# DiamondLightSource/volume-segmantics

Hardware: AMD Instinct MI355X
Metric: slices/sec fwd+bwd U-Net/ResNet-34 256x256 bf16 batch 32 (training step incl. loss, AdamW) (higher is better)
Workload: dtype bf16; 1 GPU; configs[1]: synthetic 256^3-style 1-ch slices, 2-class, U-Net/ResNet-34, batch 32 per GPU, train step (fwd + DiceLoss + bwd + AdamW + OneCycleLR); global_batch=32, slice=256x256, parallelism=dp1, master_weights=fp32

## Files before the change

### volume-segmantics_amd/csrc/conv_igemm.hip

```cpp
#include <hip/hip_fp16.h>

#include <algorithm>
#include <cstdlib>

#include "conv_common.h"
#include "conv_stream.h"
#include "prof.h"

namespace {

constexpr int kPS = 64;
__device__ __forceinline__ int swz(int row, int key, int seg) { return row * kPS + ((seg ^ ((key >> 1) & 3)) << 4); }


struct TileGeom {
    int tw_shift;
    int TH;
    int tiles_h, tiles_w;
    int PH, PW;
    int out_nchw;
    unsigned pw_magic, tw_magic;
    int groups, ctiles;
    unsigned ct_magic, ti_magic;
    unsigned long long* probe;
};

constexpr int patch_items(int pt, int stride, int nw = 4) {
    return nw == 8 ? 3 : (stride == 2 ? (pt == 2 ? 9 : 5) : (pt == 4 ? 6 : (pt == 2 ? 3 : 2)));
}

template <typename T, int BN, int PT, int NTAPS, int STRIDE, int NW = 4, int DIL = 1, bool NLOAD = false>
__global__ __launch_bounds__(NW * 64, NW == 8 ? 4 : 1) void conv_igemm_kernel(ConvParams p, TileGeom g) {
    constexpr int NT = NW * 64;
    constexpr int CK = CT<T>::CK, EPS = CT<T>::EPS;
    constexpr int NJ = BN / 16, KW = NTAPS == 9 ? 3 : 1;
    constexpr int PITEMS = patch_items(PT, DIL > 1 ? 2 : STRIDE, NW);
    constexpr int WROWS = NT / 4;
    constexpr int TS = WROWS / BN;
    static_assert(WROWS % BN == 0, "cout tile must divide the rows of a staging pass");
    constexpr int WITEMS = (NTAPS + TS - 1) / TS;
    extern __shared__ __attribute__((aligned(16))) char smem[];
    const int tid = threadIdx.x, lane = tid & 63, wave = tid >> 6;
    const int lq = lane >> 4, lr = lane & 15;
    constexpr bool kStatic = STRIDE == 1 && DIL == 1;
    constexpr int kTWS = PT == 1 ? 3 : 4, kTW = 1 << kTWS, kTH = NW * 16 * PT / kTW, kKH = NTAPS == 9 ? 3 : 1;
    const int tw_shift = kStatic ? kTWS : g.tw_shift;
    const int TW = 1 << tw_shift;
    const int PW = kStatic ? kTW - 1 + KW : g.PW;
    const int PH = kStatic ? kTH - 1 + kKH : g.PH;
    const int TH = kStatic ? kTH : g.TH;
    const int Cin = p.C0 + p.C1;
    const int P = PH * PW;
    char* patch = smem;
    char* wl = smem + P * kPS;
    asm volatile("" ::"s"(p.src0), "s"(p.src1), "s"(p.w), "s"(p.out), "s"(p.C0), "s"(p.C1), "s"(p.up0), "s"(p.Hin), "s"(p.Win),
                 "s"(p.Hout), "s"(p.Wout), "s"(p.pad), "s"(p.Cout), "s"(g.tiles_w), "s"(g.tw_magic), "s"(g.pw_magic), "s"(g.PW),
                 "s"(g.PH), "s"(g.tw_shift), "s"(g.probe), "s"(p.gc));
    unsigned long long tprobe[5];
    if (g.probe) tprobe[0] = wall_clock64();

    const int xcd = blockIdx.x & 7, slot = blockIdx.x >> 3;
    const int gl = g.ctiles == 1 ? slot : (int)__umulhi((unsigned)slot, g.ct_magic);
    const int ytile = slot - gl * g.ctiles;
    const int grp = gl * 8 + xcd;
    if (grp >= g.groups) return;
    const int tiles_img = g.tiles_h * g.tiles_w;
    const int n = tiles_img == 1 ? grp : (int)__umulhi((unsigned)grp, g.ti_magic);
    const int timg = grp - n * tiles_img;
    const int ty = g.tiles_w == 1 ? timg : (int)__umulhi((unsigned)timg, g.tw_magic);
    const int tx = timg - ty * g.tiles_w;
    const int h0 = ty * TH, w0 = tx * TW;
    const int n0 = ytile * BN;
    const int hbase = h0 * STRIDE - p.pad, wbase = w0 * STRIDE - p.pad;
    const int ush = p.up0 ? 1 : 0;
    const bool stuffed = p.up0 == 2;
    const int H0 = p.Hin >> ush, W0 = p.Win >> ush;
    const __amdgpu_buffer_rsrc_t r0 = __builtin_amdgcn_make_buffer_rsrc(
        (void*)((const T*)p.src0 + (size_t)n * H0 * W0 * p.C0), 0, H0 * W0 * p.C0 * (int)sizeof(T), 0x00020000);
    const __amdgpu_buffer_rsrc_t r1 = __builtin_amdgcn_make_buffer_rsrc(
        (void*)((const T*)p.src1 + (size_t)n * p.Hin * p.Win * p.C1), 0, p.src1 ? p.Hin * p.Win * p.C1 * (int)sizeof(T) : 0, 0x00020000);
    const int kbeg = p.gc ? n0 : 0, kend = p.gc ? n0 + p.gc : Cin;
    const int CinW = p.gc ? p.gc : Cin;
    const __amdgpu_buffer_rsrc_t rw = __builtin_amdgcn_make_buffer_rsrc((void*)p.w, 0, p.Cout * NTAPS * CinW * (int)sizeof(T), 0x00020000);
    const int dummy = (P + NTAPS * BN) * kPS;
    float* cst = reinterpret_cast<float*>(smem + dummy + 64);
    const int C0r = (p.C0 + 31) & ~31;
    if constexpr (NLOAD) {
        const long long* bins = reinterpret_cast<const long long*>(p.nl_bins);
        const double rows = (double)p.nl_rows;
        for (int ch = tid; ch < p.C0; ch += NT) {
            long long sv = 0, qv = 0;
#pragma unroll 8
// ... 94 lines not shown
                    float nm[8], na[8], nb[8];
#pragma unroll
                    for (int h = 0; h < 2; ++h) {
                        const float4 m4 = *reinterpret_cast<const float4*>(q + 4 * h), a4 = *reinterpret_cast<const float4*>(q + C0r + 4 * h),
                                     b4 = *reinterpret_cast<const float4*>(q + 2 * C0r + 4 * h);
                        nm[4 * h] = m4.x; nm[4 * h + 1] = m4.y; nm[4 * h + 2] = m4.z; nm[4 * h + 3] = m4.w;
                        na[4 * h] = a4.x; na[4 * h + 1] = a4.y; na[4 * h + 2] = a4.z; na[4 * h + 3] = a4.w;
                        nb[4 * h] = b4.x; nb[4 * h + 1] = b4.y; nb[4 * h + 2] = b4.z; nb[4 * h + 3] = b4.w;
                    }
                    const bool segok = (tid & 3) * EPS < p.C0 - c0;
#pragma unroll
                    for (int i = 0; i < PITEMS; ++i) pregs[s][i] = nl_apply8(pregs[s][i], segok && poff0[i] >= 0, nm, na, nb);
                    if (p.nl_y && ytile == (c0 / CK) % g.ctiles) {
                        const __amdgpu_buffer_rsrc_t ry = __builtin_amdgcn_make_buffer_rsrc(
                            (void*)((T*)p.nl_y + (size_t)n * H0 * W0 * p.C0), 0, H0 * W0 * p.C0 * (int)sizeof(T), 0x00020000);
#pragma unroll
                        for (int i = 0; i < PITEMS; ++i) {
                            const uint4 v = pregs[s][i];
                            __builtin_amdgcn_raw_buffer_store_b128(u32x4{v.x, v.y, v.z, v.w}, ry, (segok && ((ystore >> i) & 1u)) ? poff0[i] : (int)0x80000000,
                                                                   c0 * (int)sizeof(T), 0);
                        }
                    }
                }
            }
#pragma unroll
            for (int i = 0; i < PITEMS; ++i) *reinterpret_cast<uint4*>(patch + pdst[i]) = pregs[s][i];
#pragma unroll
            for (int i = 0; i < WITEMS; ++i) {
                const bool full = (i + 1) * TS <= NTAPS;
                const int dst = (full || wtap0 + i * TS < NTAPS) ? P * kPS + wdst0 + i * WROWS * kPS : dummy;
                *reinterpret_cast<uint4*>(smem + dst) = wregs[s][i];
            }
            __syncthreads();
            if (g.probe && c0 == kbeg) tprobe[2] = wall_clock64();
            if (c0 + PF * CK < kend) load_chunk(c0 + PF * CK, pregs[s], wregs[s]);
            uint4 wf[2][NJ], xf[2][PT];
            auto read_frags = [&](int tap, uint4 (&w)[NJ], uint4 (&x)[PT]) {
                const int kh = tap / KW, kw = tap % KW;
#pragma unroll
                for (int j = 0; j < NJ; ++j) w[j] = *reinterpret_cast<const uint4*>(wl + (tap * BN + j * 16) * kPS + wbase_l);
#pragma unroll
                for (int i = 0; i < PT; ++i) x[i] = *reinterpret_cast<const uint4*>(patch + xb[i][kw] + kh * khs);
            };
            constexpr int kMfmaPerTap = NJ * PT * (sizeof(T) == 2 ? 1 : 4);
            read_frags(0, wf[0], xf[0]);
            constexpr bool kPin = BN <= 32;
            if (kPin) __builtin_amdgcn_sched_group_barrier(0x100, NJ + PT, 0);
#pragma unroll
            for (int tap = 0; tap < NTAPS; ++tap) {
                if (tap + 1 < NTAPS) read_frags(tap + 1, wf[(tap + 1) & 1], xf[(tap + 1) & 1]);
#pragma unroll
                for (int i = 0; i < PT; ++i)
#pragma unroll
                    for (int j = 0; j < NJ; ++j) mma16<T>(acc[i][j], wf[tap & 1][j], xf[tap & 1][i]);
                if (kPin && tap + 1 < NTAPS) __builtin_amdgcn_sched_group_barrier(0x100, NJ + PT, 0);
                if (kPin) __builtin_amdgcn_sched_group_barrier(0x008, kMfmaPerTap, 0);
            }
        }
    }

    if (g.probe) tprobe[3] = wall_clock64();
    conv_epilogue<T, BN, PT, NW>(p, tw_shift, g.out_nchw, n, h0, w0, n0, grp, acc, smem);
    if (g.probe) {
        __builtin_amdgcn_s_waitcnt(0);
        tprobe[4] = wall_clock64();
        if (tid == 0) {
            unsigned long long* o = g.probe + (size_t)blockIdx.x * 8;
            for (int i = 0; i < 5; ++i) o[i] = tprobe[i];
            unsigned hw, xcc;
            asm volatile("s_getreg_b32 %0, hwreg(HW_REG_HW_ID)" : "=s"(hw));
            asm volatile("s_getreg_b32 %0, hwreg(HW_REG_XCC_ID)" : "=s"(xcc));
            o[5] = hw; o[6] = xcc; o[7] = 0;
        }
    }
}

struct DirectGeom {
    int strips_w, chunks_h, RH;
    unsigned sw_magic, ch_magic;
    int nwaves, out_nchw;
    int xcd;
};

template <typename T, int BN, int MODE>
__global__ __launch_bounds__(256, 4) void conv_direct_kernel(ConvParams p, DirectGeom g) {
    constexpr int EPS = CT<T>::EPS, NJ = BN / 16, NTAPS = 9, kD = (BN == 32 && MODE == 1) ? 2 : ((BN == 16 && MODE == 0) ? 2 : 4);
    constexpr int WTOTAL = NTAPS * BN * 4, WITEMS = (WTOTAL + 255) / 256;
    constexpr int kOob = (int)0x80000000;
    __shared__ __attribute__((aligned(16))) char wl[NTAPS * BN * kPS + 64];
    asm volatile("" ::"s"(p.src0), "s"(p.w), "s"(p.out), "s"(p.C0), "s"(p.up0), "s"(p.Hin), "s"(p.Win), "s"(p.Hout), "s"(p.Wout),
                 "s"(p.Cout), "s"(p.scale), "s"(p.shift), "s"(p.relu), "s"(p.stats_partial), "s"(g.strips_w), "s"(g.chunks_h),
                 "s"(g.RH), "s"(g.sw_magic), "s"(g.ch_magic), "s"(g.nwaves));
    const int tid = threadIdx.x, lane = tid & 63, wave = tid >> 6;
    const int lq = lane >> 4, lr = lane & 15;
    const int Cin = p.C0;
    {
        const __amdgpu_buffer_rsrc_t rw = make_rsrc(p.w, p.Cout * NTAPS * Cin * (int)sizeof(T));
#pragma unroll
        for (int i = 0; i < WITEMS; ++i) {
            const int item = tid + i * 256;
            const int row = item >> 2, seg = item & 3;
            const int tap = row / BN, nr = row % BN;
            const bool ok = item < WTOTAL && nr < p.Cout && seg * EPS < Cin;
            const uint4 v = bload(rw, ok ? ((nr * NTAPS + tap) * Cin + seg * EPS) * (int)sizeof(T) : -1, 0);
            *reinterpret_cast<uint4*>(wl + (item < WTOTAL ? swz(row, row, seg) : NTAPS * BN * kPS)) = v;
        }
    }
    __syncthreads();
    const int gw = xcd_block(g.xcd) * 4 + wave;
    if (gw >= g.nwaves) return;
    const int q = g.strips_w == 1 ? gw : (int)__umulhi((unsigned)gw, g.sw_magic);
    const int ws = gw - q * g.strips_w;
    const int n = g.chunks_h == 1 ? q : (int)__umulhi((unsigned)q, g.ch_magic);
    const int hc = q - n * g.chunks_h;
    const int w0 = ws * 16, h0 = hc * g.RH, h1 = min(p.Hout, h0 + g.RH);
    const int H0 = p.Hin >> p.up0, W0 = p.Win >> p.up0;
    const int rowbytes = W0 * p.C0 * (int)sizeof(T);
    const __amdgpu_buffer_rsrc_t rx = make_rsrc((const T*)p.src0 + (size_t)n * H0 * W0 * p.C0, H0 * rowbytes);
    int coff[3];
#pragma unroll
    for (int kw = 0; kw < 3; ++kw) {
        const int col = w0 + lr + kw - 1;
        coff[kw] = (col >= 0 && col < p.Win && lq * EPS < Cin) ? ((col >> p.up0) * p.C0 + lq * EPS) * (int)sizeof(T) : -1;
    }
    const int wbase_l = swz(lr, lr, lq);
    auto load_row = [&](int hi, uint4 (&x)[3]) {
        const bool ok = hi >= 0 && hi < p.Hin;
        const int soff = ok ? (hi >> p.up0) * rowbytes : 0;
#pragma unroll
        for (int kw = 0; kw < 3; ++kw) x[kw] = bload(rx, ok ? coff[kw] : -1, soff);
    };

    const int wo = w0 + lr;
    const bool inw = wo < p.Wout;
    __amdgpu_buffer_rsrc_t ro;
    int ooff[NJ], orow;
    if constexpr (MODE == 0) {
        ro = make_rsrc((T*)p.out + (size_t)n * p.Hout * p.Wout * p.Cout, p.Hout * p.Wout * p.Cout * (int)sizeof(T));
        orow = p.Wout * p.Cout * (int)sizeof(T);
#pragma unroll
        for (int j = 0; j < NJ; ++j) ooff[j] = (inw && j * 16 + lq * 4 < p.Cout) ? (wo * p.Cout + j * 16 + lq * 4) * (int)sizeof(T) : kOob;
    } else {
        const int Ho = p.Hout >> 1, Wo = p.Wout >> 1;
        ro = make_rsrc((T*)p.out + (size_t)n * Ho * Wo * p.Cout, Ho * Wo * p.Cout * (int)sizeof(T));
        orow = Wo * p.Cout * (int)sizeof(T);
#pragma unroll
        for (int j = 0; j < NJ; ++j)
            ooff[j] = (inw && !(lr & 1) && j * 16 + lq * 4 < p.Cout) ? ((wo >> 1) * p.Cout + j * 16 + lq * 4) * (int)sizeof(T) : kOob;
    }
    float4 sc[NJ], sh[NJ];
#pragma unroll
    for (int j = 0; j < NJ; ++j) {
        const int c = j * 16 + lq * 4;
        sc[j] = make_float4(1.f, 1.f, 1.f, 1.f); sh[j] = make_float4(0.f, 0.f, 0.f, 0.f);
        if (MODE != 1) {
            float a[4] = {1.f, 1.f, 1.f, 1.f}, b[4] = {0.f, 0.f, 0.f, 0.f};
#pragma unroll
            for (int r = 0; r < 4; ++r)
                if (c + r < p.Cout) { if (p.scale) a[r] = p.scale[c + r]; if (p.shift) b[r] = p.shift[c + r]; }
            sc[j] = make_float4(a[0], a[1], a[2], a[3]); sh[j] = make_float4(b[0], b[1], b[2], b[3]);
        }
    }
    const bool affine = MODE != 1 && (p.scale || p.shift);
    float s1[NJ][4], s2[NJ][4];
    f32x4 prev[NJ];
#pragma unroll
    for (int j = 0; j < NJ; ++j) {
        prev[j] = f32x4{0.f, 0.f, 0.f, 0.f};
#pragma unroll
        for (int r = 0; r < 4; ++r) s1[j][r] = s2[j][r] = 0.f;
    }

    f32x4 a0[NJ], a1[NJ], a2[NJ];
#pragma unroll
    for (int j = 0; j < NJ; ++j) a0[j] = a1[j] = a2[j] = f32x4{0.f, 0.f, 0.f, 0.f};
    uint4 ring[kD][3];
#pragma unroll
    for (int u = 0; u < kD; ++u) load_row(h0 - 1 + u, ring[u]);
    for (int base = h0 - 1; base <= h1; base += kD) {
#pragma unroll
        for (int u = 0; u < kD; ++u) {
            const int hi = base + u;
            if (hi > h1) break;
            int wb = wbase_l;
            if (NJ > 1 || MODE != 0) asm volatile("" : "+v"(wb));
#pragma unroll
            for (int kw = 0; kw < 3; ++kw)
#pragma unroll
                for (int j = 0; j < NJ; ++j) {
                    const uint4 w0f = *reinterpret_cast<const uint4*>(wl + ((0 * 3 + kw) * BN + j * 16) * kPS + wb);
                    const uint4 w1f = *reinterpret_cast<const uint4*>(wl + ((1 * 3 + kw) * BN + j * 16) * kPS + wb);
                    const uint4 w2f = *reinterpret_cast<const uint4*>(wl + ((2 * 3 + kw) * BN + j * 16) * kPS + wb);
                    mma16<T>(a2[j], w0f, ring[u][kw]);
                    mma16<T>(a1[j], w1f, ring[u][kw]);
                    mma16<T>(a0[j], w2f, ring[u][kw]);
                }
            load_row(hi + kD, ring[u]);
            const int h = hi - 1;
            const bool live = h >= h0;
#pragma unroll
            for (int j = 0; j < NJ; ++j) {
                if (MODE == 0 && (p.stats_partial || p.stats_bins) && live && inw) {
#pragma unroll
                    for (int r = 0; r < 4; ++r) { s1[j][r] += a0[j][r]; s2[j][r] += a0[j][r] * a0[j][r]; }
                }
                float v[4] = {a0[j][0], a0[j][1], a0[j][2], a0[j][3]};
                if constexpr (MODE == 1) {
#pragma unroll
                    for (int r = 0; r < 4; ++r) { v[r] += prev[j][r]; v[r] += __shfl_xor(v[r], 1, 64); }
                    prev[j] = a0[j];
                    const int off = (live && (h & 1)) ? ooff[j] : kOob;
                    uint2 pk;
                    if constexpr (sizeof(T) == 2) {
                        pk.x = pack2<T>(v[0], v[1]);
                        pk.y = pack2<T>(v[2], v[3]);
                        __builtin_amdgcn_raw_buffer_store_b64(__builtin_bit_cast(__attribute__((ext_vector_type(2))) unsigned int, pk), ro, off, (h >> 1) * orow, 0);
                    } else {
                        __builtin_amdgcn_raw_buffer_store_b128(u32x4{__float_as_uint(v[0]), __float_as_uint(v[1]), __float_as_uint(v[2]), __float_as_uint(v[3])}, ro, off, (h >> 1) * orow, 0);
                    }
                } else {
                    if (affine) {
                        v[0] = v[0] * sc[j].x + sh[j].x; v[1] = v[1] * sc[j].y + sh[j].y;
                        v[2] = v[2] * sc[j].z + sh[j].z; v[3] = v[3] * sc[j].w + sh[j].w;
                    }
                    if (p.relu == 1) { v[0] = fmaxf(v[0], 0.f); v[1] = fmaxf(v[1], 0.f); v[2] = fmaxf(v[2], 0.f); v[3] = fmaxf(v[3], 0.f); }
                    else if (p.relu == 2) {
#pragma unroll
                        for (int r = 0; r < 4; ++r) v[r] = v[r] / (1.f + __expf(-v[r]));
                    }
                    if constexpr (MODE == 0) {
                        const int off = live ? ooff[j] : kOob;
                        if constexpr (sizeof(T) == 2) {
                            uint2 pk;
                            pk.x = pack2<T>(v[0], v[1]);
                            pk.y = pack2<T>(v[2], v[3]);
                            __builtin_amdgcn_raw_buffer_store_b64(__builtin_bit_cast(__attribute__((ext_vector_type(2))) unsigned int, pk), ro, off, h * orow, 0);
                        } else {
                            __builtin_amdgcn_raw_buffer_store_b128(u32x4{__float_as_uint(v[0]), __float_as_uint(v[1]), __float_as_uint(v[2]), __float_as_uint(v[3])}, ro, off, h * orow, 0);
                        }
                    }
                }
            }
#pragma unroll
            for (int j = 0; j < NJ; ++j) { a0[j] = a1[j]; a1[j] = a2[j]; a2[j] = f32x4{0.f, 0.f, 0.f, 0.f}; }
        }
    }
    if (MODE == 0 && (p.stats_partial || p.stats_bins)) {
#pragma unroll
        for (int j = 0; j < NJ; ++j)
#pragma unroll
            for (int r = 0; r < 4; ++r) {
#pragma unroll
                for (int o = 1; o < 16; o <<= 1) { s1[j][r] += __shfl_xor(s1[j][r], o, 64); s2[j][r] += __shfl_xor(s2[j][r], o, 64); }
                const int c = j * 16 + lq * 4 + r;
                if (lr == 0 && c < p.Cout) {
                    if (p.stats_bins) {
                        unsigned long long* b = p.stats_bins + (size_t)(gw & (p.stats_nb - 1)) * 2 * p.Cout + c;
                        atomicAdd(b, (unsigned long long)__double2ll_rn((double)s1[j][r] * kStatScale1));
                        atomicAdd(b + p.Cout, (unsigned long long)__double2ll_rn((double)s2[j][r] * kStatScale2));
                    } else {
                        p.stats_partial[((size_t)gw * 2 + 0) * p.Cout + c] = s1[j][r];
                        p.stats_partial[((size_t)gw * 2 + 1) * p.Cout + c] = s2[j][r];
                    }
                }
            }
    }
}

template <typename T, int NK>
__global__ __launch_bounds__(256, 4) void head_dgrad_planes_kernel(const float* __restrict__ dl, const T* __restrict__ w, T* __restrict__ out, int N, int classes,
                                                                  int H, int W, int C, DirectGeom g) {
    constexpr int kOob = (int)0x80000000;
    const int tid = threadIdx.x, lane = tid & 63, wave = tid >> 6;
    const int lq = lane >> 4, lr = lane & 15;
    const int gw = blockIdx.x * 4 + wave;
    if (gw >= g.nwaves) return;
    const int q = g.strips_w == 1 ? gw : (int)__umulhi((unsigned)gw, g.sw_magic);
    const int ws = gw - q * g.strips_w;
    const int n = g.chunks_h == 1 ? q : (int)__umulhi((unsigned)q, g.ch_magic);
    const int hc = q - n * g.chunks_h;
    const int x = ws * 16 + lr, h0 = hc * g.RH, h1 = min(H, h0 + g.RH);
    const int KK = 9 * classes;
    uint4 af[NK];
    int poff[NK][8];
    int prow[NK][8];
#pragma unroll
    for (int qq = 0; qq < NK; ++qq) {
        unsigned short a8[8];
#pragma unroll
        for (int j = 0; j < 8; ++j) {
            const int kk = 32 * qq + 8 * lq + j;
            const bool live = kk < KK;
            const int t = live ? kk / classes : 0, k = live ? kk - t * classes : 0;
            const int r = t / 3, sft = t - 3 * r;
            a8[j] = (live && lr < C) ? __builtin_bit_cast(unsigned short, w[((size_t)k * 9 + t) * C + lr]) : (unsigned short)0;
            const int xx = x + 1 - sft;
            poff[qq][j] = (live && xx >= 0 && xx < W) ? k * H * W + (1 - r) * W + xx : kOob;
            prow[qq][j] = r;
        }
        af[qq] = make_uint4((unsigned)a8[0] | ((unsigned)a8[1] << 16), (unsigned)a8[2] | ((unsigned)a8[3] << 16),
                            (unsigned)a8[4] | ((unsigned)a8[5] << 16), (unsigned)a8[6] | ((unsigned)a8[7] << 16));
    }
    const float* dn = dl + (size_t)n * classes * H * W;
    const __amdgpu_buffer_rsrc_t ro = make_rsrc(out + (size_t)n * H * W * C, H * W * C * (int)sizeof(T));
    const int ooff = (x < W && lq * 4 < C) ? (x * C + lq * 4) * (int)sizeof(T) : kOob;
    auto gather = [&](int y, float (&v)[NK][8]) {
        bool rok[3];
#pragma unroll
        for (int r = 0; r < 3; ++r) { const int yy = y + 1 - r; rok[r] = yy >= 0 && yy < H && y < h1; }
#pragma unroll
        for (int qq = 0; qq < NK; ++qq)
#pragma unroll
            for (int j = 0; j < 8; ++j) {
                const bool ok = poff[qq][j] != kOob && rok[prow[qq][j]];
                v[qq][j] = ok ? dn[(size_t)y * W + poff[qq][j]] : 0.f;
            }
    };
    float cur[NK][8], nxt[NK][8];
    gather(h0, cur);
    for (int y = h0; y < h1; ++y) {
        gather(y + 1, nxt);
        f32x4 acc = f32x4{0.f, 0.f, 0.f, 0.f};
#pragma unroll
        for (int qq = 0; qq < NK; ++qq) {
            uint4 b;
            b.x = pack2<T>(cur[qq][0], cur[qq][1]); b.y = pack2<T>(cur[qq][2], cur[qq][3]);
            b.z = pack2<T>(cur[qq][4], cur[qq][5]); b.w = pack2<T>(cur[qq][6], cur[qq][7]);
            mma16<T>(acc, af[qq], b);
        }
        uint2 pk;
        pk.x = pack2<T>(acc[0], acc[1]);
        pk.y = pack2<T>(acc[2], acc[3]);
        __builtin_amdgcn_raw_buffer_store_b64(__builtin_bit_cast(__attribute__((ext_vector_type(2))) unsigned int, pk), ro, ooff, y * W * C * (int)sizeof(T), 0);
#pragma unroll
        for (int qq = 0; qq < NK; ++qq)
#pragma unroll
            for (int j = 0; j < 8; ++j) cur[qq][j] = nxt[qq][j];
    }
}
// ... 190 lines not shown
        coff[kw] = (col >= 0 && col < p.Win && lq * EPS < Cin) ? (col * p.C0 + lq * EPS) * (int)sizeof(T) : -1;
    }
    auto load_row = [&](int hi, uint4 (&x)[3]) {
        const bool ok = hi >= 0 && hi < p.Hin;
        const int soff = ok ? hi * rowbytes : 0;
#pragma unroll
        for (int kw = 0; kw < 3; ++kw) x[kw] = bload(rx, ok ? coff[kw] : -1, soff);
    };
    const int wbase_l = swz(lr, lr, lq);
    const int wo = w0 + lr;
    const bool inw = wo < p.Wout;
    float bias[4];
#pragma unroll
    for (int r = 0; r < 4; ++r) bias[r] = (p.shift && r < K) ? p.shift[r] : 0.f;
    const int plane = p.Hout * p.Wout * 4;
    const __amdgpu_buffer_rsrc_t ro = MODE == 2 ? make_rsrc((float*)p.out + (size_t)n * K * p.Hout * p.Wout, K * plane) : make_rsrc(nullptr, 0);

    f32x4 acc = f32x4{0.f, 0.f, 0.f, 0.f}, done = f32x4{0.f, 0.f, 0.f, 0.f};
    uint4 ring[kD][3];
#pragma unroll
    for (int u = 0; u < kD; ++u) load_row(h0 - 1 + u, ring[u]);
    for (int base = h0 - 1; base <= h1r; base += kD) {
#pragma unroll
        for (int u = 0; u < kD; ++u) {
            const int hi = base + u;
            if (hi > h1r) break;
            const int m = (u + 3) & 3;
            int wb = wbase_l;
            asm volatile("" : "+v"(wb));
#pragma unroll
            for (int kw = 0; kw < 3; ++kw)
                mma16<T>(acc, *reinterpret_cast<const uint4*>(wl + (m * 3 + kw) * 16 * kPS + wb), ring[u][kw]);
            load_row(hi + kD, ring[u]);
            const int qd = (u + 2) & 3;
            if (lq == qd) { done = acc; acc = f32x4{0.f, 0.f, 0.f, 0.f}; }
            if (qd == 3) {
                const int h = hi - 4 + lq;
                const bool live = h >= h0 && h < h1 && inw;
                float v[4];
#pragma unroll
                for (int r = 0; r < 4; ++r) v[r] = done[r] + bias[r];
                if constexpr (MODE == 2) {
#pragma unroll
                    for (int r = 0; r < 4; ++r)
                        __builtin_amdgcn_raw_buffer_store_b32(__float_as_uint(v[r]), ro, (live && r < K) ? (h * p.Wout + wo) * 4 : kOob, r * plane, 0);
                } else {
                    float mx = v[0];
#pragma unroll
                    for (int r = 1; r < 4; ++r) if (r < K) mx = fmaxf(mx, v[r]);
                    float sum = 0.f;
#pragma unroll
                    for (int r = 0; r < 4; ++r) if (r < K) sum += expf(v[r] - mx);
                    float best = -1.f;
                    int lab = 0;
#pragma unroll
                    for (int r = 0; r < 4; ++r)
                        if (r < K) { const float pk = __fdiv_rn(expf(v[r] - mx), sum); if (pk > best) { best = pk; lab = r; } }
                    const int rr = h - vsc.m.crop_top, jj = wo - vsc.m.crop_left;
                    if (live && rr >= 0 && rr < vsc.m.h && jj >= 0 && jj < vsc.m.w) {
                        const int64_t addr = vsc.m.base + (int64_t)(vsc.s0 + n) * vsc.m.ss + (int64_t)rr * vsc.m.sh + (int64_t)jj * vsc.m.sw;
                        const __half hv = __float2half_rn(best);
                        const uint32_t hb = __builtin_bit_cast(uint16_t, hv);
                        if (vsc.mode == 0) {
                            if (vsc.labels) vsc.labels[addr] = (uint8_t)lab;
                            if (vsc.probs) vsc.probs[addr] = (uint16_t)hb;
                        } else if (!vsc.stage) {
                            atomicMax(vsc.keys + addr, (hb << 16) | ((uint32_t)(15 - vsc.direction) << 8) | (uint32_t)lab);
                        } else {
                            vsc.stage[((int64_t)n * p.Hout + h) * p.Wout + wo] = (hb << 16) | ((uint32_t)(15 - vsc.direction) << 8) | (uint32_t)lab;
                        }
                    }
                }
            }
        }
    }
}

static bool direct_ok(int dtype, const ConvParams& p) {
    const int CK = dtype == VS_F32 ? 16 : 32;
    const bool nchw = (p.out_f32 >> 1) != 0, f32 = (p.out_f32 & 1) != 0;
    const bool head_ok = p.Cout <= 4 && !p.pool0 && !p.scale && !p.relu && !p.up0 && !p.stats_partial;
    const bool out_ok = p.scatter ? (head_ok && (p.scatter->mode == 0 || (p.scatter->mode == 1 && p.scatter->keys)))
                                  : nchw ? (f32 && head_ok) : (!f32 && !(p.Cout & 3));
    return vs_option("conv_direct") && out_ok && !p.nl_bins && !p.bz && !p.gc && p.dil <= 1 && p.up0 != 2 && p.KH == 3 && p.KW == 3 && p.stride == 1 && p.pad == 1 && p.C1 == 0 && p.C0 <= CK &&
           p.Cout <= 16 && !p.residual && !p.out1 && (!p.pool0 || (!(p.Hout & 1) && !(p.Wout & 1) && p.Cout % 4 == 0)) &&
           (long)p.N * p.Hout * p.Wout >= (long)vs_option("conv_direct_min_px") &&
           (double)p.Hout * p.Wout * std::max(p.Cout, 4) * 4.0 < 2.0e9;
}
static DirectGeom direct_geom(const ConvParams& p) {
    DirectGeom g{};
    g.strips_w = cdiv(p.Wout, 16);
    const bool big = (long)p.N * p.Hout * p.Wout >= (4L << 20) * 4;
    g.RH = std::max(2, vs_option(big ? "conv_direct_rows_big" : "conv_direct_rows") & ~1);
    g.chunks_h = cdiv(p.Hout, g.RH);
    g.sw_magic = 0xffffffffu / (unsigned)g.strips_w + 1u;
    g.ch_magic = 0xffffffffu / (unsigned)g.chunks_h + 1u;
    g.nwaves = p.N * g.strips_w * g.chunks_h;
    g.xcd = 0;
    return g;
}

template <typename T, int BN>
int launch_direct(const ConvParams& p, int out_nchw, hipStream_t s) {
    DirectGeom g = direct_geom(p);
    g.out_nchw = out_nchw;
    VS_REQUIRE((double)p.Hin * p.Win * p.C0 * sizeof(T) < 2.0e9 && (long)g.nwaves * 16 < (1L << 32), "conv_direct: tensor too large");
    const bool head = p.scatter || (p.Cout & 3) != 0 || out_nchw;
    if (head) {
        g.RH = std::max(4, g.RH & ~3);
        g.chunks_h = cdiv(p.Hout, g.RH);
        g.ch_magic = 0xffffffffu / (unsigned)g.chunks_h + 1u;
        g.nwaves = p.N * g.strips_w * g.chunks_h;
        VS_REQUIRE(!p.up0 && !p.relu && !p.scale && !p.stats_partial, "conv_head: plain 3x3 head only");
    }
    const dim3 grid(cdiv(g.nwaves, 4));
    const size_t pad = 0;
    VolScatter sc{};
    if (p.scatter) {
        sc = *p.scatter;
        ConvParams q = p;
        q.scatter = nullptr;
        hipLaunchKernelGGL((conv_head_kernel<T, 3>), grid, dim3(256), pad, s, q, g, sc);
    } else if (head) {
        VS_REQUIRE(out_nchw && p.Cout <= 4 && BN == 16 && !p.pool0 && !p.scale, "conv_direct: unsupported ragged output");
        hipLaunchKernelGGL((conv_head_kernel<T, 2>), grid, dim3(256), pad, s, p, g, sc);
    } else if (p.pool0) {
        hipLaunchKernelGGL((conv_direct_kernel<T, BN, 1>), grid, dim3(256), pad, s, p, g);
    } else {
        VS_REQUIRE(!p.out_f32, "conv_direct: fp32 NHWC output is not supported");
        hipLaunchKernelGGL((conv_direct_kernel<T, BN, 0>), grid, dim3(256), pad, s, p, g);
    }
    VS_LAUNCH_CHECK();
    return VS_OK;
}

static DirectGeom pair_geom(const ConvParams& q) {
    DirectGeom g{};
    g.strips_w = cdiv(q.Wout, 14);
    const bool big = (long)q.N * q.Hout * q.Wout >= (4L << 20) * 4;
    g.RH = std::max(2, vs_option(big ? "conv_direct_rows_big" : "conv_direct_rows") & ~1);
    g.chunks_h = cdiv(q.Hout, g.RH);
    g.sw_magic = 0xffffffffu / (unsigned)g.strips_w + 1u;
    g.ch_magic = 0xffffffffu / (unsigned)g.chunks_h + 1u;
    g.nwaves = q.N * g.strips_w * g.chunks_h;
    return g;
}

template <typename T, int BN, int PT, int NTAPS, int STRIDE, int NW = 4, int DIL = 1, bool NLOAD = false>
int launch_one(const ConvParams& p, const TileGeom& g, hipStream_t s) {
    static bool attr_set = false;
    auto kern = conv_igemm_kernel<T, BN, PT, NTAPS, STRIDE, NW, DIL, NLOAD>;
    const size_t lds = (size_t)g.PH * g.PW * kPS + (size_t)NTAPS * BN * kPS + 64 + (NLOAD ? (size_t)3 * ((p.C0 + 31) & ~31) * sizeof(float) : 0);
    VS_REQUIRE((double)p.Hin * p.Win * std::max(p.C0, p.C1) * sizeof(T) < 2.0e9 && (double)p.Cout * NTAPS * (p.C0 + p.C1) * sizeof(T) < 2.0e9,
               "conv_igemm: image or weight tensor exceeds the 32-bit staging offsets");
    VS_REQUIRE(lds <= 160 * 1024, "conv_igemm: LDS request %zu too large", lds);
    VS_REQUIRE(g.PH * g.PW * 4 <= patch_items(PT, DIL > 1 ? 2 : STRIDE, NW) * NW * 64, "conv_igemm: patch %dx%d exceeds the staging budget", g.PH, g.PW);
    if (!attr_set) {
        VS_CHECK_HIP(hipFuncSetAttribute((const void*)kern, hipFuncAttributeMaxDynamicSharedMemorySize, 160 * 1024));
        attr_set = true;
    }
    VS_REQUIRE(g.tiles_h * g.tiles_w < 65536 && p.N < 65536 && g.PH * g.PW + NW * 64 < 65536, "conv_igemm: tile grid too large");
    TileGeom gg = g;
    gg.groups = p.N * g.tiles_h * g.tiles_w;
    gg.ctiles = cdiv(p.Cout, BN);
    gg.ct_magic = 0xffffffffu / (unsigned)gg.ctiles + 1u;
    gg.ti_magic = 0xffffffffu / (unsigned)(g.tiles_h * g.tiles_w) + 1u;
    const long nwg = (long)cdiv(gg.groups, 8) * 8 * gg.ctiles;
    VS_REQUIRE(nwg < (1L << 31) && (long)gg.groups * (g.tiles_h * g.tiles_w) < (1L << 32), "conv_igemm: tile grid too large");
    if (g.probe) gg.probe = vs_probe_buffer((size_t)nwg);
    hipLaunchKernelGGL(kern, dim3((unsigned)nwg), dim3(NW * 64), lds, s, p, gg);
    VS_LAUNCH_CHECK();
    return VS_OK;
}

struct Pick { int BN, PT, NW; };
static int tile_tw(const ConvParams& p, int PT) { return p.stride == 1 ? (PT == 1 ? 8 : 16) : (p.Wout >= 16 ? 16 : 8); }

Pick pick_cfg(const ConvParams& p) {
    Pick c;
    c.NW = 4;
    c.PT = (p.stride == 1 && p.Hout * p.Wout >= 128 && p.Wout >= 16) ? 2 : 1;
    if (p.stride == 2 && p.KH == 3 && p.Cout >= 64 && !p.gc && p.Wout >= 16 && p.Hout >= 8 &&
        (long)p.N * cdiv(p.Hout, 8) * cdiv(p.Wout, 16) * cdiv(p.Cout, 64) >= vs_option("conv_min_wgs")) c.PT = 2;
    const bool can8 = vs_option("conv_nw8") && p.stride == 1 && p.dil <= 1 && p.Hout >= 16 && p.Wout >= 16;
    auto wgs = [&](int bn, int px) {
        const int tw = tile_tw(p, px == 64 ? 1 : 2), th = px / tw;
        return (long)p.N * cdiv(p.Hout, th) * cdiv(p.Wout, tw) * cdiv(p.Cout, bn);
    };
    int bn = p.Cout >= 64 ? 64 : (p.Cout >= 32 ? 32 : 16);
    if (p.gc) bn = 32;
    if (p.out1 && p.split_c % 64 != 0 && bn == 64) bn = 32;
    if (p.out1 && p.split_c % 32 != 0 && bn == 32) bn = 16;
    if (can8 && wgs(bn, 256) >= vs_option("conv_nw8_min_wgs")) { c.NW = 8; c.PT = 2; }
    if (bn == 64 && wgs(64, c.NW * c.PT * 16) < vs_option("conv_min_wgs")) bn = 32;
    c.BN = bn;
    return c;
}

static int stream_mode(int dtype, const ConvParams& p, int out_nchw) {
    if ((dtype != VS_BF16 && dtype != VS_F16) || !vs_option("conv_stream") || !ring::stream_ok(p, out_nchw) || p.C0 + p.C1 > 512 || p.nl_bins) return 0;
    const int bn = (p.Cout % 64 == 0) ? 64 : 32;
    const long jobs = (long)p.N * cdiv(p.Hout, 16) * cdiv(p.Wout, 16) * (p.Cout / bn);
    return jobs >= 256L * vs_option("conv_stream_min_tiles") ? bn : 0;
}

static int ring_mode(int dtype, const ConvParams& p, int out_nchw) {
    if (dtype != VS_BF16 || !vs_option("conv_ring") || p.KH != 3 || p.KW != 3 || p.stride != 1 || p.pad != 1 || p.dil > 1 || p.gc || p.scatter ||
        out_nchw || (p.Cout & 3) || p.out_f32) return 0;
    if (p.nl_bins && ((p.C0 & 31) || p.up0 == 2 || p.C0 > 1024)) return 0;
    const int Cin = p.C0 + p.C1;
// ... 219 lines not shown
```

### volume-segmantics_amd/csrc/unet.hip

```cpp
#include <cstdlib>
#include <cmath>
#include <string>
#include <vector>

#include "common.h"
#include "prof.h"

namespace {

struct TensorInfo {
    std::string name;
    int64_t shape[4];
    int ndim, kind;
    int64_t offset;
};

enum UnitKind { U_STEM, U_POOL, U_CONV, U_HEAD, U_CONCAT,
                U_CONVT,
                U_ADD,
                U_UPADD,
                U_BILINEAR,
                U_DROPOUT,
                U_DWCONV,
                U_GAP,
// ... 2178 lines not shown
            dzp = c.dz(u.out); dz_c = u.cout;
            if (u.kind == U_CONV && u.bias_idx >= 0) {
                if ((rc = vs_colsum(dt, dzp, c.rows(u), u.cout, grads + c.t(u.bias_idx).offset, (float*)(c.ws + net->off_bnws), net->bnws_bytes, stream))) return rc;
            }
            if (u.kind == U_CONVT) {
                ProfScope prof(PK_POOL_MISC, 0, 3.0 * n * u.hout * u.wout * u.cout * net->esz, c.s);
                if ((rc = vs_colsum(dt, dzp, c.rows(u), u.cout, grads + c.t(u.bias_idx).offset, (float*)(c.ws + net->off_bnws), net->bnws_bytes, stream))) return rc;
                if ((rc = vs_space_to_depth2(dt, dzp, c.da(u.out), n, u.hin, u.win, u.cout, stream))) return rc;
                dzp = c.da(u.out); dz_c = 4 * u.cout;
            }
        }
        pending.push_back(SideItem{ui, dzp, dz_c});
        const bool flush = (int)pending.size() >= fork_every || ui == unit_lo || u.kind == U_STEM;
        if (flush && do_main && (rc = fork_mark(ui))) return rc;
        if (u.colr && do_main) {
            ConvParams p{};
            p.src0 = dzp; p.C0 = u.cout; p.N = n; p.Hin = p.Hout = u.hin; p.Win = p.Wout = u.win; p.stride = 1; p.pad = 0; p.KH = p.KW = 1;
            p.w = c.ws + Ctx::wt_off(u, net->wset); p.Cout = 9 * u.cin0; p.out = c.ws + net->off_ys;
            {
                ProfScope prof(PK_CONV_DGRAD, conv_flops(c, u), 0, c.s);
                if ((rc = launch_conv_igemm(dt, p, c.s))) return rc;
            }
            if ((rc = vs_dilated_im2col(dt, p.out, c.da(u.src0), n, u.hin, u.win, u.cin0, u.colr, 1, written[u.src0] ? 1 : 0, stream))) return rc;
            written[u.src0] = 1;
        } else if (u.kind == U_DWCONV2 && do_main) {
            if (!u.bcast) {
                ProfScope prof(PK_CONV_DGRAD, 2.0 * n * u.hout * u.wout * u.cout * u.k * u.k, 0, c.s);
                if ((rc = vs_dwconv2d_bwd_data(dt, dzp, c.P(u.w_idx), c.da(u.src0), n, u.hin, u.win, u.cout, u.k, u.stride, u.pad, u.dil, u.hout, u.wout,
                                               written[u.src0] ? 1 : 0, stream))) return rc;
                written[u.src0] = 1;
            }
        } else if (u.kind == U_DWCONV && do_main) {
            ProfScope prof(PK_CONV_DGRAD, 2.0 * n * u.hout * u.wout * u.cout * 9, 0, c.s);
            if ((rc = vs_dwconv3x3(dt, dzp, c.P(u.w_idx), c.da(u.src0), n, u.hin, u.win, u.cout, u.dil, 1 | (written[u.src0] ? 2 : 0), stream))) return rc;
            written[u.src0] = 1;
        } else if (u.kind == U_HEAD && head_planes && do_main) {
            ProfScope prof(PK_CONV_DGRAD, 2.0 * n * u.hout * u.wout * net->classes * u.k * u.k * u.cin0, 0, c.s);
            if ((rc = launch_head_dgrad_planes(dt, head_dl, c.ws + Ctx::wc_off(u, net->wset), c.da(u.src0), n, net->classes, u.hout, u.wout, u.cin0, c.s))) return rc;
            written[u.src0] = 1;
        } else if (u.kind != U_STEM && do_main) {
        ConvParams p{};
        const void* dsrc = dzp;
        const bool stuff_in_loader = u.stride == 2 && !(u.hin & 1) && !(u.win & 1);
        if (u.stride == 2 && !stuff_in_loader) {
            void* zs = c.ws + net->off_zs;
            ProfScope prof(PK_POOL_MISC, 0, (double)n * u.hin * u.win * dz_c * net->esz * 1.25, c.s);
            if ((rc = vs_zero_stuff2x(dt, dzp, zs, n, u.hout, u.wout, dz_c, stream))) return rc;
            dsrc = zs;
        }
        p.src0 = dsrc; p.C0 = dz_c; p.N = n; p.Hin = u.hin; p.Win = u.win; p.Hout = u.hin; p.Wout = u.win;
        if (stuff_in_loader) p.up0 = 2;
        p.stride = 1; p.pad = u.pad; p.KH = p.KW = u.k;
        p.w = c.ws + Ctx::wt_off(u, net->wset); p.Cout = u.cin0 + u.cin1;
        p.gc = u.cg ? 32 : 0;
        p.dil = u.dil;
        if (u.up0) {
            const bool acc0 = written[u.src0] != 0;
            VS_REQUIRE(u.src1 < 0 || !written[u.src1], "backward: decoder skip gradient written twice");
            if (u.src1 >= 0) { p.out1 = c.da(u.src1); p.split_c = u.cin0; written[u.src1] = 1; }
            if (!acc0 && conv_plan(dt, p).can_pool) {
                p.pool0 = 1;
                p.out = c.da(u.src0);
                const ConvPlan plan = conv_plan(dt, p);
                prof_set_variant(plan.code);
                ProfScope prof(PK_CONV_DGRAD, conv_flops(c, u), 0, c.s);
                prof_set_variant(0);
                if ((rc = launch_conv_igemm(dt, p, c.s, &plan))) return rc;
            } else {
                p.out = c.ws + net->off_dup;
                {
                    ProfScope prof(PK_CONV_DGRAD, conv_flops(c, u), 0, c.s);
                    if ((rc = launch_conv_igemm(dt, p, c.s))) return rc;
                }
                ProfScope prof(PK_POOL_MISC, 0, (double)n * u.hin * u.win * u.cin0 * net->esz * 1.25, c.s);
                if ((rc = launch_upsample2x_bwd(dt, p.out, c.da(u.src0), n, u.hin / 2, u.win / 2, u.cin0, acc0 ? 1 : 0, c.s))) return rc;
            }
            written[u.src0] = 1;
        } else {
            p.out = c.da(u.src0);
            p.residual = written[u.src0] ? c.da(u.src0) : nullptr;
            const int pa = u.src0, pu = net->producer[pa];
            ConvPlan plan = conv_plan(dt, p);
            if (vs_option("fuse_bn_bwd") && pu >= 0 && pu == ui - 1 && net->first_consumer[pa] == ui && net->units[pu].kind == U_CONV &&
                net->units[pu].bn_idx >= 0 && !(p.Cout & 3) && plan.family != CONV_DIRECT) {
                const Unit& q = net->units[pu];
                const int rows_needed = plan.stat_rows;
                if ((size_t)rows_needed * 2 * q.cout * sizeof(float) <= net->bnws_bytes) {
                    const bool recompute = q.relu && q.res < 0;
                    p.bz = c.z(q.out);
                    p.by = (q.relu && !recompute) ? c.a(q.out) : nullptr;
                    p.bmean = c.bnc(q, 2); p.binvstd = c.bnc(q, 3);
                    p.bgamma = c.P(q.bn_idx); p.bbeta = c.P(q.bn_idx + 1);
                    p.bstats_partial = (float*)(c.ws + net->off_bnws);
                    p.brelu = q.relu;
                    net->bwd_stat_rows[pa] = rows_needed;
                    plan = conv_plan(dt, p);
                }
            }
            prof_set_variant(plan.code);
            ProfScope prof(PK_CONV_DGRAD, u.kind == U_HEAD ? 2.0 * n * u.hout * u.wout * net->classes * u.k * u.k * u.cin0 : conv_flops(c, u), 0, c.s);
            prof_set_variant(0);
            if ((rc = launch_conv_igemm(dt, p, c.s, &plan))) return rc;
            written[u.src0] = 1;
        }
        }
        if (flush) {
            if (do_side) {
                if ((rc = fork_wait(ui))) return rc;
                for (const SideItem& it : pending) {
                    if (stem_on_caller && net->units[it.ui].kind == U_STEM) {
                        hipStream_t keep_s = ws_stream;
                        float* keep_w = wgws;
                        ws_stream = c.s;
                        wgws = (float*)(c.ws + net->off_wgws + net->wgws_bytes);
                        rc = side_wgrad(it);
                        ws_stream = keep_s; wgws = keep_w;
                        if (rc) return rc;
                        continue;
                    }
                    if ((rc = side_wgrad(it))) return rc;
                }
            }
            pending.clear();
            prof_set_tag(ui);
        }
    }
    if (!pending.empty()) {
        const int ui = pending.back().ui;
        if (do_main && (rc = fork_mark(ui))) return rc;
        if (do_side) {
            if ((rc = fork_wait(ui))) return rc;
            for (const SideItem& it : pending)
                if ((rc = side_wgrad(it))) return rc;
        }
        pending.clear();
    }
    if (use_side) {
        for (int i = 0; i < vs_unet::kSide; ++i) {
            if (!side_used[i]) continue;
            VS_CHECK_HIP(hipEventRecord(net->join_event[i], net->side[i]));
            VS_CHECK_HIP(hipStreamWaitEvent(c.s, net->join_event[i], 0));
        }
    }
    if (opt && role == ROLE_BOTH) net->wset ^= 1;
    return VS_OK;
}

extern "C" int vs_unet_backward_adamw(vs_unet_t* net, const float* x, const float* dlogits, int n, int need_encoder_wgrad,
                                      float* grads, void* workspace, void* stream, const vs_adamw_args* opt) {
    VS_REQUIRE(net && opt && opt->params && opt->exp_avg && opt->exp_avg_sq && opt->step >= 1, "unet_backward_adamw: bad optimiser arguments");
    return unet_backward_range(net, opt->params, x, dlogits, n, need_encoder_wgrad, grads, workspace, stream, 0,
                               (int)net->units.size(), opt);
}

extern "C" int vs_unet_backward_adamw_part(vs_unet_t* net, const float* x, const float* dlogits, int n, int need_encoder_wgrad,
                                           float* grads, void* workspace, void* stream, const vs_adamw_args* opt, int unit_lo,
                                           int unit_hi, int role) {
    VS_REQUIRE(net && opt && opt->params && opt->exp_avg && opt->exp_avg_sq && opt->step >= 1, "unet_backward_adamw_part: bad optimiser arguments");
    VS_REQUIRE(unit_lo >= 0 && unit_lo < unit_hi && unit_hi <= (int)net->units.size(), "unet_backward_adamw_part: bad unit range");
    VS_REQUIRE(role == ROLE_MAIN || role == ROLE_SIDE, "unet_backward_adamw_part: role must be 1 (caller's stream) or 2 (weight gradients)");
    return unet_backward_range(net, opt->params, x, dlogits, n, need_encoder_wgrad, grads, workspace, stream, unit_lo, unit_hi, opt, role);
}

extern "C" int vs_unet_backward_part(vs_unet_t* net, const float* params, const float* x, const float* dlogits, int n,
                                     int need_encoder_wgrad, float* grads, void* workspace, void* stream, int unit_lo,
                                     int unit_hi, int role) {
    VS_REQUIRE(net && unit_lo >= 0 && unit_lo < unit_hi && unit_hi <= (int)net->units.size(), "unet_backward_part: bad unit range");
    VS_REQUIRE(role == ROLE_MAIN || role == ROLE_SIDE, "unet_backward_part: role must be 1 (caller's stream) or 2 (weight gradients)");
    return unet_backward_range(net, params, x, dlogits, n, need_encoder_wgrad, grads, workspace, stream, unit_lo, unit_hi, nullptr, role);
}

extern "C" int vs_unet_adamw_range(vs_unet_t* net, int need_encoder_wgrad, const float* grads, void* workspace, void* stream,
                                   const vs_adamw_args* opt, int unit_lo, int unit_hi) {
    VS_REQUIRE(net && grads && workspace && opt && opt->params && opt->exp_avg && opt->exp_avg_sq && opt->step >= 1,
               "unet_adamw_range: bad arguments");
    VS_REQUIRE(unit_lo >= 0 && unit_lo < unit_hi && unit_hi <= (int)net->units.size(), "unet_adamw_range: bad unit range");
    Ctx c{net, (char*)workspace, opt->params, nullptr, (hipStream_t)stream, net->last_n};
    return update_units(c, unit_lo, unit_hi, need_encoder_wgrad != 0, grads, *opt, (hipStream_t)stream);
}
// ... 109 lines not shown
```

Before: 7219 slices/s.

## Fuse BN-backward epilogue into the direct 3x3 conv dgrad kernel

Adds a BZ variant of the direct conv kernel that, in its dgrad epilogue, reloads the producer's pre-BN activations, recomputes the ReLU mask, and accumulates the BN backward partial sums before storing the masked gradient. The planner now also allows the fused BN-backward path when the dgrad conv uses the direct family. This is meant to remove a separate BN-backward/ReLU-mask pass over the small-channel (16-cout) layers. In exchange, each row does an extra z load and some epilogue arithmetic, which may raise register pressure in the direct kernel.

```diff
diff --git a/volume-segmantics_amd/csrc/conv_igemm.hip b/volume-segmantics_amd/csrc/conv_igemm.hip
--- a/volume-segmantics_amd/csrc/conv_igemm.hip
+++ b/volume-segmantics_amd/csrc/conv_igemm.hip
@@ -8,6 +8,7 @@
 #include "prof.h"
 
 namespace {
+using ring::u32x2;
 
 constexpr int kPS = 64;
 __device__ __forceinline__ int swz(int row, int key, int seg) { return row * kPS + ((seg ^ ((key >> 1) & 3)) << 4); }
@@ -268,8 +269,9 @@
     int xcd;
 };
 
-template <typename T, int BN, int MODE>
+template <typename T, int BN, int MODE, bool BZ = false>
 __global__ __launch_bounds__(256, 4) void conv_direct_kernel(ConvParams p, DirectGeom g) {
+    static_assert(!BZ || (BN == 16 && MODE == 0 && !std::is_same<T, f16_t>::value), "the BN-backward epilogue is built for the 16-cout NHWC form (bf16 / fp32)");
     constexpr int EPS = CT<T>::EPS, NJ = BN / 16, NTAPS = 9, kD = (BN == 32 && MODE == 1) ? 2 : ((BN == 16 && MODE == 0) ? 2 : 4);
     constexpr int WTOTAL = NTAPS * BN * 4, WITEMS = (WTOTAL + 255) / 256;
     constexpr int kOob = (int)0x80000000;
@@ -357,6 +359,27 @@
         for (int r = 0; r < 4; ++r) s1[j][r] = s2[j][r] = 0.f;
     }
 
+    typedef typename std::conditional<sizeof(T) == 2, u32x2, u32x4>::type zraw_t;
+    __amdgpu_buffer_rsrc_t rz = ro;
+    float bmu[4] = {0.f, 0.f, 0.f, 0.f}, bis[4] = {0.f, 0.f, 0.f, 0.f}, bga[4] = {0.f, 0.f, 0.f, 0.f}, bbe[4] = {0.f, 0.f, 0.f, 0.f};
+    zraw_t zcur{}, znxt{};
+    if constexpr (BZ) {
+        rz = make_rsrc((const T*)p.bz + (size_t)n * p.Hout * p.Wout * p.Cout, p.Hout * p.Wout * p.Cout * (int)sizeof(T));
+#pragma unroll
+        for (int r = 0; r < 4; ++r) {
+            const int c = lq * 4 + r;
+            if (c < p.Cout) {
+                bmu[r] = p.bmean[c]; bis[r] = p.binvstd[c];
+                if (p.brelu) { bga[r] = bis[r] * p.bgamma[c]; bbe[r] = p.bbeta[c]; }
+            }
+        }
+    }
+    auto load_z = [&](int h) -> zraw_t {
+        const bool ok = h >= h0 && h < h1;
+        if constexpr (sizeof(T) == 2) return __builtin_amdgcn_raw_buffer_load_b64(rz, ok ? ooff[0] : kOob, ok ? h * orow : 0, 0);
+        else return __builtin_amdgcn_raw_buffer_load_b128(rz, ok ? ooff[0] : kOob, ok ? h * orow : 0, 0);
+    };
+
     f32x4 a0[NJ], a1[NJ], a2[NJ];
 #pragma unroll
     for (int j = 0; j < NJ; ++j) a0[j] = a1[j] = a2[j] = f32x4{0.f, 0.f, 0.f, 0.f};
@@ -369,7 +392,7 @@
             const int hi = base + u;
             if (hi > h1) break;
             int wb = wbase_l;
-            if (NJ > 1 || MODE != 0) asm volatile("" : "+v"(wb));
+            if (NJ > 1 || MODE != 0 || BZ) asm volatile("" : "+v"(wb));
 #pragma unroll
             for (int kw = 0; kw < 3; ++kw)
 #pragma unroll
@@ -381,9 +404,36 @@
                     mma16<T>(a1[j], w1f, ring[u][kw]);
                     mma16<T>(a0[j], w2f, ring[u][kw]);
                 }
+            if constexpr (BZ) { zcur = znxt; znxt = load_z(hi); }
             load_row(hi + kD, ring[u]);
             const int h = hi - 1;
             const bool live = h >= h0;
+            if constexpr (BZ) {
+                const float av[4] = {a0[0][0], a0[0][1], a0[0][2], a0[0][3]};
+                const float4 gq = ld4_roundtrip<T>(av);
+                float gv[4] = {gq.x, gq.y, gq.z, gq.w}, zv[4];
+                if constexpr (sizeof(T) == 2) {
+                    zv[0] = __uint_as_float(zcur[0] << 16); zv[1] = __uint_as_float(zcur[0] & 0xffff0000u);
+                    zv[2] = __uint_as_float(zcur[1] << 16); zv[3] = __uint_as_float(zcur[1] & 0xffff0000u);
+                } else {
+#pragma unroll
+                    for (int r = 0; r < 4; ++r) zv[r] = __uint_as_float(zcur[r]);
+                }
+                if (p.brelu) {
+#pragma unroll
+                    for (int r = 0; r < 4; ++r) gv[r] = ((zv[r] - bmu[r]) * bga[r] + bbe[r]) > 0.f ? gv[r] : 0.f;
+                }
+                if (live && inw) {
+#pragma unroll
+                    for (int r = 0; r < 4; ++r) { s1[0][r] += gv[r]; s2[0][r] += gv[r] * (zv[r] - bmu[r]) * bis[r]; }
+                }
+                const int off = live ? ooff[0] : kOob;
+                if constexpr (sizeof(T) == 2) {
+                    __builtin_amdgcn_raw_buffer_store_b64(u32x2{pack2<T>(gv[0], gv[1]), pack2<T>(gv[2], gv[3])}, ro, off, h * orow, 0);
+                } else {
+                    __builtin_amdgcn_raw_buffer_store_b128(u32x4{__float_as_uint(gv[0]), __float_as_uint(gv[1]), __float_as_uint(gv[2]), __float_as_uint(gv[3])}, ro, off, h * orow, 0);
+                }
+            } else {
 #pragma unroll
             for (int j = 0; j < NJ; ++j) {
                 if (MODE == 0 && (p.stats_partial || p.stats_bins) && live && inw) {
@@ -427,11 +477,12 @@
                     }
                 }
             }
+            }
 #pragma unroll
             for (int j = 0; j < NJ; ++j) { a0[j] = a1[j]; a1[j] = a2[j]; a2[j] = f32x4{0.f, 0.f, 0.f, 0.f}; }
         }
     }
-    if (MODE == 0 && (p.stats_partial || p.stats_bins)) {
+    if (MODE == 0 && (BZ || p.stats_partial || p.stats_bins)) {
 #pragma unroll
         for (int j = 0; j < NJ; ++j)
 #pragma unroll
@@ -440,7 +491,10 @@
                 for (int o = 1; o < 16; o <<= 1) { s1[j][r] += __shfl_xor(s1[j][r], o, 64); s2[j][r] += __shfl_xor(s2[j][r], o, 64); }
                 const int c = j * 16 + lq * 4 + r;
                 if (lr == 0 && c < p.Cout) {
-                    if (p.stats_bins) {
+                    if constexpr (BZ) {
+                        p.bstats_partial[((size_t)gw * 2 + 0) * p.Cout + c] = s1[j][r];
+                        p.bstats_partial[((size_t)gw * 2 + 1) * p.Cout + c] = s2[j][r];
+                    } else if (p.stats_bins) {
                         unsigned long long* b = p.stats_bins + (size_t)(gw & (p.stats_nb - 1)) * 2 * p.Cout + c;
                         atomicAdd(b, (unsigned long long)__double2ll_rn((double)s1[j][r] * kStatScale1));
                         atomicAdd(b + p.Cout, (unsigned long long)__double2ll_rn((double)s2[j][r] * kStatScale2));
@@ -797,7 +851,9 @@
     const bool head_ok = p.Cout <= 4 && !p.pool0 && !p.scale && !p.relu && !p.up0 && !p.stats_partial;
     const bool out_ok = p.scatter ? (head_ok && (p.scatter->mode == 0 || (p.scatter->mode == 1 && p.scatter->keys)))
                                   : nchw ? (f32 && head_ok) : (!f32 && !(p.Cout & 3));
-    return vs_option("conv_direct") && out_ok && !p.nl_bins && !p.bz && !p.gc && p.dil <= 1 && p.up0 != 2 && p.KH == 3 && p.KW == 3 && p.stride == 1 && p.pad == 1 && p.C1 == 0 && p.C0 <= CK &&
+    const bool bz_ok = !p.bz || (!p.by && !p.pool0 && !p.scale && !p.shift && !p.relu && !p.scatter && !nchw && !f32 && !p.stats_partial && !p.stats_bins &&
+                                 dtype != VS_F16);
+    return vs_option("conv_direct") && out_ok && !p.nl_bins && bz_ok && !p.gc && p.dil <= 1 && p.up0 != 2 && p.KH == 3 && p.KW == 3 && p.stride == 1 && p.pad == 1 && p.C1 == 0 && p.C0 <= CK &&
            p.Cout <= 16 && !p.residual && !p.out1 && (!p.pool0 || (!(p.Hout & 1) && !(p.Wout & 1) && p.Cout % 4 == 0)) &&
            (long)p.N * p.Hout * p.Wout >= (long)vs_option("conv_direct_min_px") &&
            (double)p.Hout * p.Wout * std::max(p.Cout, 4) * 4.0 < 2.0e9;
@@ -841,6 +897,14 @@
         hipLaunchKernelGGL((conv_head_kernel<T, 2>), grid, dim3(256), pad, s, p, g, sc);
     } else if (p.pool0) {
         hipLaunchKernelGGL((conv_direct_kernel<T, BN, 1>), grid, dim3(256), pad, s, p, g);
+    } else if (p.bz) {
+        if constexpr (BN == 16 && !std::is_same<T, f16_t>::value) {
+            VS_REQUIRE(!p.out_f32 && !p.by, "conv_direct: the BN-backward epilogue recomputes its mask and stores NHWC in the storage type");
+            hipLaunchKernelGGL((conv_direct_kernel<T, BN, 0, true>), grid, dim3(256), pad, s, p, g);
+        } else {
+            vs_set_error("conv_direct: no BN-backward epilogue for this dtype");
+            return VS_ERR_UNSUPPORTED;
+        }
     } else {
         VS_REQUIRE(!p.out_f32, "conv_direct: fp32 NHWC output is not supported");
         hipLaunchKernelGGL((conv_direct_kernel<T, BN, 0>), grid, dim3(256), pad, s, p, g);
diff --git a/volume-segmantics_amd/csrc/unet.hip b/volume-segmantics_amd/csrc/unet.hip
--- a/volume-segmantics_amd/csrc/unet.hip
+++ b/volume-segmantics_amd/csrc/unet.hip
@@ -2284,19 +2284,22 @@
             const int pa = u.src0, pu = net->producer[pa];
             ConvPlan plan = conv_plan(dt, p);
             if (vs_option("fuse_bn_bwd") && pu >= 0 && pu == ui - 1 && net->first_consumer[pa] == ui && net->units[pu].kind == U_CONV &&
-                net->units[pu].bn_idx >= 0 && !(p.Cout & 3) && plan.family != CONV_DIRECT) {
+                net->units[pu].bn_idx >= 0 && !(p.Cout & 3)) {
                 const Unit& q = net->units[pu];
-                const int rows_needed = plan.stat_rows;
-                if ((size_t)rows_needed * 2 * q.cout * sizeof(float) <= net->bnws_bytes) {
-                    const bool recompute = q.relu && q.res < 0;
-                    p.bz = c.z(q.out);
-                    p.by = (q.relu && !recompute) ? c.a(q.out) : nullptr;
-                    p.bmean = c.bnc(q, 2); p.binvstd = c.bnc(q, 3);
-                    p.bgamma = c.P(q.bn_idx); p.bbeta = c.P(q.bn_idx + 1);
-                    p.bstats_partial = (float*)(c.ws + net->off_bnws);
-                    p.brelu = q.relu;
+                const bool recompute = q.relu && q.res < 0;
+                ConvParams pb = p;
+                pb.bz = c.z(q.out);
+                pb.by = (q.relu && !recompute) ? c.a(q.out) : nullptr;
+                pb.bmean = c.bnc(q, 2); pb.binvstd = c.bnc(q, 3);
+                pb.bgamma = c.P(q.bn_idx); pb.bbeta = c.P(q.bn_idx + 1);
+                pb.bstats_partial = (float*)(c.ws + net->off_bnws);
+                pb.brelu = q.relu;
+                const ConvPlan bplan = conv_plan(dt, pb);
+                const int rows_needed = bplan.stat_rows;
+                if ((plan.family != CONV_DIRECT || bplan.family == CONV_DIRECT) && (size_t)rows_needed * 2 * q.cout * sizeof(float) <= net->bnws_bytes) {
+                    p = pb;
+                    plan = bplan;
                     net->bwd_stat_rows[pa] = rows_needed;
-                    plan = conv_plan(dt, p);
                 }
             }
             prof_set_variant(plan.code);
```

Result: no change. 7212 slices/s (-0.1%).
